# korneelvdbroek/audiocodec

Measured on AMD Instinct MI355X. Metric: MDCT frames/s (48 kHz, N=1024) encode+decode, higher is better.
Workload: dtype f32

## Files before the change

audiocodec_amd/csrc/ac_fast_inv.hip:

```cpp
#include "ac_fast_inv_dev.h"

namespace ac {

int pick_seglen(long long pairs, int frames, int preferred) {
  static const int fixed = [] {
    const char* e = getenv("AC_SEGLEN");
    return e ? atoi(e) : 0;
  }();
  int s = fixed > 0 ? fixed : preferred;
  if (s > frames) s = frames;
  if (s < 1) s = 1;
  return s;
}

template <int R, int IOF>
static void launch_inv_R(const InvArgs& a, int C, unsigned grid, hipStream_t s) {
  const dim3 blk(AC_WAVES * 64);
  if (C == 2) hipLaunchKernelGGL((k_inv_fast<R, 0, AC_WAVES, IOF>), dim3(grid), blk, 0, s, a);
  else if (C == 1) hipLaunchKernelGGL((k_inv_fast<R, 2, AC_WAVES, IOF>), dim3(grid), blk, 0, s, a);
  else if constexpr (IOF != 2) hipLaunchKernelGGL((k_inv_fast<R, 1, AC_WAVES, IOF>), dim3(grid), blk, 0, s, a);
}

int launch_inv_fast(const ac_mdct_plan* p, const float* X, void* x, int iof, const float* tail_in, float* tail_out,
                    int B, int Kp, int nblk, int C, hipStream_t s) {
  if (B <= 0 || C <= 0 || nblk <= 0) return AC_OK;
  if (fast_mdct_frames_per_wave(p->N) > 1) {
    if (!fast_multi_serves(p, C, iof, Kp)) {
      set_error("internal: no wave-level synthesis kernel for filters_n = %d, %d channels, io format %d here", p->N, C, iof);
      return AC_EUNSUPPORTED;
    }
    return launch_inv_multi(p, X, x, iof, tail_in, tail_out, B, Kp, nblk, C, s);
  }
  InvArgs a;
  unsigned grid;
  const int st = prep_inv_fast(p, X, x, iof, tail_in, tail_out, B, Kp, nblk, C, a, grid);
  if (st) return st;
  if (p->N == Geo<8>::FN) {
    if (iof == 2) launch_inv_R<8, 2>(a, C, grid, s);
    else if (iof == 1) launch_inv_R<8, 1>(a, C, grid, s);
    else launch_inv_R<8, 0>(a, C, grid, s);
  } else if (iof == 2) launch_inv_R<16, 2>(a, C, grid, s);
  else if (iof == 1) launch_inv_R<16, 1>(a, C, grid, s);
  else launch_inv_R<16, 0>(a, C, grid, s);
  AC_HIP_CHECK(hipGetLastError());
  return AC_OK;
}

bool fast_inv_quant_serves(const ac_mdct_plan* p, int C) {
  return p->fast && fast_mdct_frames_per_wave(p->N) == 1 && (C == 1 || C == 2);
}

template <int R, int IOF>
static void launch_inv_q_R(const InvArgs& a, const QuantRows& qr, int C, unsigned grid, hipStream_t s) {
  const dim3 blk(AC_WAVES * 64);
  if (C == 2) hipLaunchKernelGGL((k_inv_fast_q<R, 0, AC_WAVES, IOF>), dim3(grid), blk, 0, s, a, qr);
  else hipLaunchKernelGGL((k_inv_fast_q<R, 2, AC_WAVES, IOF>), dim3(grid), blk, 0, s, a, qr);
}

int launch_inv_fast_quant(const ac_mdct_plan* p, const ac_psy_plan* psy, const int16_t* codes, const int8_t* sf, void* x,
                          bool pcm16, int B, int Kp, int C, hipStream_t s) {
  if (B <= 0 || C <= 0 || Kp <= 0) return AC_OK;
  if (!fast_inv_quant_serves(p, C) || psy->N != p->N) {
    set_error("internal: no synthesis from quantised spectra for filters_n = %d, %d channels", p->N, C);
    return AC_EUNSUPPORTED;
  }
  InvArgs a;
  unsigned grid;
  const int st = prep_inv_fast(p, reinterpret_cast<const float*>(codes), x, pcm16 ? 1 : 0, nullptr, nullptr, B, Kp, Kp + 1, C,
                               a, grid);
  if (st) return st;
  QuantRows qr;
  qr.sf = sf;
  qr.band32 = reinterpret_cast<const uint32_t*>(psy->d_qband);
  qr.M = psy->M;
  if (p->N == Geo<8>::FN) {
    if (pcm16) launch_inv_q_R<8, 4>(a, qr, C, grid, s);
    else launch_inv_q_R<8, 3>(a, qr, C, grid, s);
  } else if (pcm16) launch_inv_q_R<16, 4>(a, qr, C, grid, s);
  else launch_inv_q_R<16, 3>(a, qr, C, grid, s);
  AC_HIP_CHECK(hipGetLastError());
  return AC_OK;
}

}
```

audiocodec_amd/csrc/ac_fast_inv_dev.h:

```cpp
#pragma once
#include <cstdlib>

#include "ac_fast.h"
#include "ac_fast_dev.h"

namespace ac {
namespace {

struct InvArgs {
  const float* X;
  void* x;
  const float* tail_in;
  float* tail_out;
  const float* tab;
  int B, Kp, nblk, C, seglen, nseg;
  int rev;
  long long npairs, nsig;
  long long ntasks;
};

template <int R>
__device__ __forceinline__ void idct_frame(const v4f (&frm)[R], char* buf, gtab_t tab, const v2f (&p1)[R], int lane,
                                           v2f (&now)[R], v2f (&nxt)[R]) {
  using G = Geo<R>;
  C2 z[R];
  {
    v2f xo_in[R], xo[R];
#pragma unroll
    for (int c = 0; c < R; ++c) xo_in[c] = v2f{frm[c].z, frm[c].w};
    rev_exchange<R - 1, R>(buf, lane, xo_in, xo);
#pragma unroll
    for (int r = 0; r < R; ++r) {
      const C2 v = {v2f{frm[r].x, frm[r].y}, xo[r]};
      z[r] = cmul(v, reinterpret_cast<const v2f*>(tab + G::I_PRE)[r * 64 + lane]);
    }
  }
  fft_wave<R>(z, buf, tab, p1, lane);
#pragma unroll
  for (int j = 0; j < R; ++j) {
    const C2 r = cmul_negim(z[j], reinterpret_cast<const v2f*>(tab + G::I_POST)[j * 64 + lane]);
    if (j < R / 2) {
      now[j] = r.re;
      nxt[j] = r.im;
    } else {
      now[j] = r.im;
      nxt[j] = r.re;
    }
  }
}

struct QuantRows {
  const int8_t* sf;
  const uint32_t* band32;
  int M;
};

template <int R, int CMODE, int NW, int IOF = 0>
__device__ __forceinline__ void inv_fast_body(const InvArgs& a, char* lds, const int bid, const int nblocks,
                                              const QuantRows* qr = nullptr) {
  using G = Geo<R>;
  constexpr bool QUANT = IOF >= 3;
  constexpr int OIOF = QUANT ? IOF - 3 : IOF;
  constexpr int FH = G::FH;
  const int lane = threadIdx.x & 63, wave = __builtin_amdgcn_readfirstlane(threadIdx.x >> 6);
  load_tables<NW, WAVE_LDS, G::I_LDS, 0>(lds, a.tab + G::I_TOTAL, nullptr);
  char* buf = lds + wave * WAVE_LDS;
  gtab_t tab = reinterpret_cast<const float*>(lds + NW * WAVE_LDS);
  v2f p1[R];
  load_p1<R>(a.tab + G::I_TOTAL, lane, p1);
  const int C = a.C;
  const size_t blk = (size_t)G::FN * C;
  constexpr bool COOP = (R == 8);
  const long long task_raw = (long long)(a.rev ? nblocks - 1 - bid : bid) * NW + wave;
  const bool valid = task_raw < a.ntasks;
  const long long task = valid ? task_raw : a.ntasks - 1;
  const int sgm = (int)(task % a.nseg);
  const Pair pq = make_pair<CMODE>(task / a.nseg, C, a.nsig);
  const bool has1 = pq.has1;
  const int n0 = sgm * a.seglen;
  const int n1 = min(a.nblk, n0 + a.seglen);
  using spec_t = typename std::conditional<IOF == 2 || QUANT, int16_t, float>::type;
  const spec_t* X0 = reinterpret_cast<const spec_t*>(a.X) + row_off(pq.b0, a.Kp, 0, blk, pq.c0);
  const spec_t* X1 = reinterpret_cast<const spec_t*>(a.X) + row_off(pq.b1, a.Kp, 0, blk, pq.c1);
  using hold_t = typename std::conditional<QUANT, QGran, v4f>::type;
  constexpr bool BW_REGS = QUANT && R == 8;
  uint32_t bw[BW_REGS ? R : 1];
  if constexpr (BW_REGS) {
#pragma unroll
    for (int i = 0; i < R; ++i) bw[i] = qr->band32[64 * i + lane];
  }
  auto load_frame = [&](int n, const spec_t* r0, const spec_t* r1, hold_t (&dst)[R]) {
    if constexpr (QUANT) {
      const size_t mc = (size_t)qr->M * C;
      const int8_t* sf0 = qr->sf + row_off(pq.b0, a.Kp, n, mc, pq.c0);
      const int8_t* sf1 = qr->sf + row_off(pq.b1, a.Kp, n, mc, pq.c1);
      if constexpr (BW_REGS) {
        load_row_q<CMODE, R>(r0, r1, sf0, sf1, bw, has1, lane, dst);
      } else {
        uint32_t bl[R];
#pragma unroll
        for (int i = 0; i < R; ++i) bl[i] = qr->band32[64 * i + lane];
        load_row_q<CMODE, R>(r0, r1, sf0, sf1, bl, has1, lane, dst);
      }
    } else if constexpr (IOF == 2) load_row_h<Bf16Fmt, CMODE, R>(r0, r1, C, has1, lane, dst);
    else load_row<CMODE, R>(r0, r1, C, has1, lane, dst);
  };
  const size_t ts0 = ((size_t)pq.b0 * C + pq.c0) * FH, ts1 = ((size_t)pq.b1 * C + pq.c1) * FH;
  constexpr bool AHEAD = (R == 8);
  const bool left = valid && n0 >= 1;
  const bool deferred = COOP && left && wave > 0;

  auto emit = [&](int n, const v2f (&now)[R], const v2f (&cin)[R]) {
    v4f row[R];
    v2f xe[R], xo_in[R], xo[R];
#pragma unroll
    for (int j2 = 0; j2 < R; ++j2) {
      const v2f ab = reinterpret_cast<const v2f*>(tab + G::I_COEF)[j2 * 64 + lane];
      const v2f o1 = ab.x * now[j2] + ab.y * cin[j2];
      const v2f o2 = ab.y * now[j2] - ab.x * cin[j2];
      xe[(j2 + R / 2) & (R - 1)] = (j2 < R / 2) ? o2 : o1;
      xo_in[j2] = (j2 < R / 2) ? o1 : o2;
    }
    rev_exchange<R / 2 - 1, R>(buf, lane, xo_in, xo);
#pragma unroll
    for (int i = 0; i < R; ++i) row[i] = v4f{xe[i].x, xe[i].y, xo[i].x, xo[i].y};
    const size_t o0 = row_off(pq.b0, a.nblk, n, blk, pq.c0), o1 = row_off(pq.b1, a.nblk, n, blk, pq.c1);
    if constexpr (OIOF != 0)
      store_row_h<typename RowFmt<OIOF>::type, CMODE, R>(static_cast<int16_t*>(a.x) + o0, static_cast<int16_t*>(a.x) + o1, C, has1, lane, row);
    else store_row<CMODE, R>(static_cast<float*>(a.x) + o0, static_cast<float*>(a.x) + o1, C, has1, lane, row);
  };

  v2f carry[R], now0[R];
#pragma unroll
  for (int r = 0; r < R; ++r) {
    carry[r] = v2f{0.f, 0.f};
    now0[r] = v2f{0.f, 0.f};
  }
  if (valid) {
    hold_t ahead[R];
    if (left && !deferred) {
      hold_t row[R];
      load_frame(n0 - 1, X0 + (size_t)(n0 - 1) * blk, X1 + (size_t)(n0 - 1) * blk, row);
      if (AHEAD && n0 < a.Kp) load_frame(n0, X0 + (size_t)n0 * blk, X1 + (size_t)n0 * blk, ahead);
      v2f dummy[R];
      if constexpr (QUANT) {
        v4f frm[R];
        dequant_frame<R>(row, frm);
        idct_frame<R>(frm, buf, tab, p1, lane, dummy, carry);
      } else {
        idct_frame<R>(row, buf, tab, p1, lane, dummy, carry);
      }
    } else {
      if (AHEAD && n0 < a.Kp) load_frame(n0, X0 + (size_t)n0 * blk, X1 + (size_t)n0 * blk, ahead);
      if (!left && a.tail_in) {
#pragma unroll
        for (int j2 = 0; j2 < R; ++j2) {
          const int k = lane + 64 * j2;
          const int j = (j2 < R / 2) ? (FH - 1 - 2 * k) : (2 * k - FH);
          carry[j2].x = a.tail_in[ts0 + j];
          carry[j2].y = has1 ? a.tail_in[ts1 + j] : 0.f;
        }
      }
    }

    for (int n = n0; n < n1; ++n) {
      v2f now[R], nxt[R];
      if (n < a.Kp) {
        if (!AHEAD) load_frame(n, X0 + (size_t)n * blk, X1 + (size_t)n * blk, ahead);
        if constexpr (QUANT) {
          v4f frm[R];
          dequant_frame<R>(ahead, frm);
          idct_frame<R>(frm, buf, tab, p1, lane, now, nxt);
        } else {
          idct_frame<R>(ahead, buf, tab, p1, lane, now, nxt);
        }
        if (AHEAD && n + 1 < n1 && n + 1 < a.Kp)
          load_frame(n + 1, X0 + (size_t)(n + 1) * blk, X1 + (size_t)(n + 1) * blk, ahead);
      } else {
#pragma unroll
        for (int r = 0; r < R; ++r) {
          now[r] = v2f{0.f, 0.f};
          nxt[r] = v2f{0.f, 0.f};
        }
      }
      if (deferred && n == n0) {
#pragma unroll
        for (int r = 0; r < R; ++r) now0[r] = now[r];
      } else {
        emit(n, now, carry);
      }
#pragma unroll
      for (int r = 0; r < R; ++r) carry[r] = nxt[r];
    }

    if (a.tail_out && n1 == a.nblk) {
#pragma unroll
      for (int j2 = 0; j2 < R; ++j2) {
        const int k = lane + 64 * j2;
        const int j = (j2 < R / 2) ? (FH - 1 - 2 * k) : (2 * k - FH);
        a.tail_out[ts0 + j] = carry[j2].x;
        if (has1) a.tail_out[ts1 + j] = carry[j2].y;
      }
    }
  }

  if (COOP) {
    wave_sync();
    if (valid) {
#pragma unroll
      for (int r = 0; r < R; ++r) *reinterpret_cast<v2f*>(buf + 8 * lane + 512 * r) = carry[r];
    }
    __syncthreads();
    v2f cin[R];
    if (deferred) {
#pragma unroll
      for (int r = 0; r < R; ++r) cin[r] = *reinterpret_cast<const v2f*>(buf - WAVE_LDS + 8 * lane + 512 * r);
    }
    __syncthreads();
    if (deferred) emit(n0, now0, cin);
  }
}

template <int R, int CMODE, int NW, int IOF = 0>
__global__ __launch_bounds__(NW * 64, ((IOF == 2 || (IOF == 1 && !(R == 8 && CMODE != 1))) ? 2 : wpe<R, CMODE>())) void k_inv_fast(InvArgs a) {
  __shared__ __attribute__((aligned(16))) char lds[NW * WAVE_LDS + Geo<R>::TAB_LDS];
  inv_fast_body<R, CMODE, NW, IOF>(a, lds, (int)blockIdx.x, (int)gridDim.x);
}

template <int R, int CMODE, int NW, int IOF>
__global__ __launch_bounds__(NW * 64, 2) void k_inv_fast_q(InvArgs a, QuantRows qr) {
  static_assert(IOF == 3 || IOF == 4, "quantised spectra");
  __shared__ __attribute__((aligned(16))) char lds[NW * WAVE_LDS + Geo<R>::TAB_LDS];
  inv_fast_body<R, CMODE, NW, IOF>(a, lds, (int)blockIdx.x, (int)gridDim.x, &qr);
}

static int prep_inv_fast(const ac_mdct_plan* p, const float* X, void* x, int iof, const float* tail_in, float* tail_out,
                         int B, int Kp, int nblk, int C, InvArgs& a, unsigned& grid) {
  if (iof == 2 && C > 2) {
    set_error("internal: no wave-level synthesis kernel for bfloat16 tensors with %d channels", C);
    return AC_EUNSUPPORTED;
  }
  a.X = X;
  a.x = x;
  a.tail_in = tail_in;
  a.tail_out = tail_out;
  a.tab = p->d_fast;
  a.B = B;
  a.Kp = Kp;
  a.nblk = nblk;
  a.C = C;
  a.nsig = (long long)B * C;
  a.npairs = (C == 2) ? (long long)B : (a.nsig + 1) / 2;
  a.seglen = pick_seglen(a.npairs, nblk, (p->N == Geo<8>::FN && C == 2) ? 2 : 3);
  if (a.npairs * ((nblk + a.seglen - 1) / a.seglen) < (long long)AC_WAVES * p->cus * 2) a.seglen = pick_seglen(a.npairs, nblk, 1);
  a.nseg = (nblk + a.seglen - 1) / a.seglen;
  a.ntasks = a.npairs * a.nseg;
  static const int inv_rev = [] { const char* e = getenv("AC_INV_REV"); return e ? atoi(e) : 0; }();
  a.rev = inv_rev;
  return grid_for(a.ntasks, AC_WAVES, &grid);
}

}
}
```

Before: 284.6 million.

## Let inverse MDCT blocks loop over several task rounds with carry hand-off

Each workgroup of the N=1024 inverse kernel now processes T rounds of tasks. The overlap carry of the last wave is handed to wave 0 of the next round through LDS, so wave 0 can skip recomputing the previous frame. The goal is to amortise table loading and the redundant left-frame IDCT across rounds, using a smaller grid. With the default of one round, behaviour is essentially unchanged apart from the restructured loop, extra registers (hand, pinned p1) and asm barriers.

```diff
diff --git a/audiocodec_amd/csrc/ac_fast_inv.hip b/audiocodec_amd/csrc/ac_fast_inv.hip
--- a/audiocodec_amd/csrc/ac_fast_inv.hip
+++ b/audiocodec_amd/csrc/ac_fast_inv.hip
@@ -11,6 +11,17 @@
   if (s > frames) s = frames;
   if (s < 1) s = 1;
   return s;
+}
+
+constexpr int INV_ROUNDS = 1;
+static int set_inv_rounds(const ac_mdct_plan* p, InvArgs& a, unsigned& grid) {
+  if (p->N != Geo<8>::FN) return AC_OK;
+  const char* e = getenv("AC_INV_ROUNDS");
+  int T = e ? atoi(e) : 0;
+  if (T <= 0) T = INV_ROUNDS;
+  if (T > 64) T = 64;
+  a.T = T;
+  return grid_for((a.ntasks + T - 1) / T, AC_WAVES, &grid);
 }
 
 template <int R, int IOF>
@@ -33,7 +44,8 @@
   }
   InvArgs a;
   unsigned grid;
-  const int st = prep_inv_fast(p, X, x, iof, tail_in, tail_out, B, Kp, nblk, C, a, grid);
+  int st = prep_inv_fast(p, X, x, iof, tail_in, tail_out, B, Kp, nblk, C, a, grid);
+  if (!st) st = set_inv_rounds(p, a, grid);
   if (st) return st;
   if (p->N == Geo<8>::FN) {
     if (iof == 2) launch_inv_R<8, 2>(a, C, grid, s);
@@ -66,8 +78,8 @@
   }
   InvArgs a;
   unsigned grid;
-  const int st = prep_inv_fast(p, reinterpret_cast<const float*>(codes), x, pcm16 ? 1 : 0, nullptr, nullptr, B, Kp, Kp + 1, C,
-                               a, grid);
+  int st = prep_inv_fast(p, reinterpret_cast<const float*>(codes), x, pcm16 ? 1 : 0, nullptr, nullptr, B, Kp, Kp + 1, C, a, grid);
+  if (!st) st = set_inv_rounds(p, a, grid);
   if (st) return st;
   QuantRows qr;
   qr.sf = sf;
diff --git a/audiocodec_amd/csrc/ac_fast_inv_dev.h b/audiocodec_amd/csrc/ac_fast_inv_dev.h
--- a/audiocodec_amd/csrc/ac_fast_inv_dev.h
+++ b/audiocodec_amd/csrc/ac_fast_inv_dev.h
@@ -15,9 +15,15 @@
   const float* tab;
   int B, Kp, nblk, C, seglen, nseg;
   int rev;
+  int T;
   long long npairs, nsig;
   long long ntasks;
 };
+
+template <typename V>
+__device__ __forceinline__ void per_round(V& v) {
+  asm volatile("" : "+v"(v));
+}
 
 template <int R>
 __device__ __forceinline__ void idct_frame(const v4f (&frm)[R], char* buf, gtab_t tab, const v2f (&p1)[R], int lane,
@@ -62,7 +68,8 @@
   constexpr bool QUANT = IOF >= 3;
   constexpr int OIOF = QUANT ? IOF - 3 : IOF;
   constexpr int FH = G::FH;
-  const int lane = threadIdx.x & 63, wave = __builtin_amdgcn_readfirstlane(threadIdx.x >> 6);
+  int lane = threadIdx.x & 63;
+  const int wave = __builtin_amdgcn_readfirstlane(threadIdx.x >> 6);
   load_tables<NW, WAVE_LDS, G::I_LDS, 0>(lds, a.tab + G::I_TOTAL, nullptr);
   char* buf = lds + wave * WAVE_LDS;
   gtab_t tab = reinterpret_cast<const float*>(lds + NW * WAVE_LDS);
@@ -71,17 +78,12 @@
   const int C = a.C;
   const size_t blk = (size_t)G::FN * C;
   constexpr bool COOP = (R == 8);
-  const long long task_raw = (long long)(a.rev ? nblocks - 1 - bid : bid) * NW + wave;
-  const bool valid = task_raw < a.ntasks;
-  const long long task = valid ? task_raw : a.ntasks - 1;
-  const int sgm = (int)(task % a.nseg);
-  const Pair pq = make_pair<CMODE>(task / a.nseg, C, a.nsig);
-  const bool has1 = pq.has1;
-  const int n0 = sgm * a.seglen;
-  const int n1 = min(a.nblk, n0 + a.seglen);
+  const int T = COOP ? a.T : 1;
+  const long long first = (long long)(a.rev ? nblocks - 1 - bid : bid) * (NW * T);
+  const int nmine = (int)min(a.ntasks - first, (long long)(NW * T));
+  const long long pair0 = first / a.nseg;
+  const unsigned sgm0 = (unsigned)(first - pair0 * a.nseg);
   using spec_t = typename std::conditional<IOF == 2 || QUANT, int16_t, float>::type;
-  const spec_t* X0 = reinterpret_cast<const spec_t*>(a.X) + row_off(pq.b0, a.Kp, 0, blk, pq.c0);
-  const spec_t* X1 = reinterpret_cast<const spec_t*>(a.X) + row_off(pq.b1, a.Kp, 0, blk, pq.c1);
   using hold_t = typename std::conditional<QUANT, QGran, v4f>::type;
   constexpr bool BW_REGS = QUANT && R == 8;
   uint32_t bw[BW_REGS ? R : 1];
@@ -89,135 +91,179 @@
 #pragma unroll
     for (int i = 0; i < R; ++i) bw[i] = qr->band32[64 * i + lane];
   }
-  auto load_frame = [&](int n, const spec_t* r0, const spec_t* r1, hold_t (&dst)[R]) {
-    if constexpr (QUANT) {
-      const size_t mc = (size_t)qr->M * C;
-      const int8_t* sf0 = qr->sf + row_off(pq.b0, a.Kp, n, mc, pq.c0);
-      const int8_t* sf1 = qr->sf + row_off(pq.b1, a.Kp, n, mc, pq.c1);
-      if constexpr (BW_REGS) {
-        load_row_q<CMODE, R>(r0, r1, sf0, sf1, bw, has1, lane, dst);
+  constexpr bool AHEAD = (R == 8);
+  auto pin_p1 = [&]() {
+    if constexpr (COOP) {
+#pragma unroll
+      for (int k = 1; k < R; ++k) per_round(p1[k]);
+    }
+  };
+  v2f hand[R];
+#pragma unroll
+  for (int r = 0; r < R; ++r) hand[r] = v2f{0.f, 0.f};
+
+  for (int t = 0; t < T; ++t) {
+    per_round(lane);
+    const int mine = t * NW + wave;
+    const bool valid = mine < nmine;
+    const unsigned ofs = sgm0 + (unsigned)(valid ? mine : nmine - 1);
+    const unsigned dp = ofs / (unsigned)a.nseg;
+    const int sgm = (int)(ofs - dp * (unsigned)a.nseg);
+    const Pair pq = make_pair<CMODE>(pair0 + dp, C, a.nsig);
+    const bool has1 = pq.has1;
+    const int n0 = sgm * a.seglen;
+    const int n1 = min(a.nblk, n0 + a.seglen);
+    const spec_t* X0 = reinterpret_cast<const spec_t*>(a.X) + row_off(pq.b0, a.Kp, 0, blk, pq.c0);
+    const spec_t* X1 = reinterpret_cast<const spec_t*>(a.X) + row_off(pq.b1, a.Kp, 0, blk, pq.c1);
+    auto load_frame = [&](int n, const spec_t* r0, const spec_t* r1, hold_t (&dst)[R]) {
+      if constexpr (QUANT) {
+        const size_t mc = (size_t)qr->M * C;
+        const int8_t* sf0 = qr->sf + row_off(pq.b0, a.Kp, n, mc, pq.c0);
+        const int8_t* sf1 = qr->sf + row_off(pq.b1, a.Kp, n, mc, pq.c1);
+        if constexpr (BW_REGS) {
+          load_row_q<CMODE, R>(r0, r1, sf0, sf1, bw, has1, lane, dst);
+        } else {
+          uint32_t bl[R];
+#pragma unroll
+          for (int i = 0; i < R; ++i) bl[i] = qr->band32[64 * i + lane];
+          load_row_q<CMODE, R>(r0, r1, sf0, sf1, bl, has1, lane, dst);
+        }
+      } else if constexpr (IOF == 2) load_row_h<Bf16Fmt, CMODE, R>(r0, r1, C, has1, lane, dst);
+      else load_row<CMODE, R>(r0, r1, C, has1, lane, dst);
+    };
+    const size_t ts0 = ((size_t)pq.b0 * C + pq.c0) * FH, ts1 = ((size_t)pq.b1 * C + pq.c1) * FH;
+    const bool left = valid && n0 >= 1;
+    const bool deferred = COOP && left && wave > 0;
+    const bool handed = COOP && left && wave == 0 && t > 0;
+
+    auto emit = [&](int n, const v2f (&now)[R], const v2f (&cin)[R]) {
+      v4f row[R];
+      v2f xe[R], xo_in[R], xo[R];
+#pragma unroll
+      for (int j2 = 0; j2 < R; ++j2) {
+        const v2f ab = reinterpret_cast<const v2f*>(tab + G::I_COEF)[j2 * 64 + lane];
+        const v2f o1 = ab.x * now[j2] + ab.y * cin[j2];
+        const v2f o2 = ab.y * now[j2] - ab.x * cin[j2];
+        xe[(j2 + R / 2) & (R - 1)] = (j2 < R / 2) ? o2 : o1;
+        xo_in[j2] = (j2 < R / 2) ? o1 : o2;
+      }
+      rev_exchange<R / 2 - 1, R>(buf, lane, xo_in, xo);
+#pragma unroll
+      for (int i = 0; i < R; ++i) row[i] = v4f{xe[i].x, xe[i].y, xo[i].x, xo[i].y};
+      const size_t o0 = row_off(pq.b0, a.nblk, n, blk, pq.c0), o1 = row_off(pq.b1, a.nblk, n, blk, pq.c1);
+      if constexpr (OIOF != 0)
+        store_row_h<typename RowFmt<OIOF>::type, CMODE, R>(static_cast<int16_t*>(a.x) + o0, static_cast<int16_t*>(a.x) + o1, C, has1, lane, row);
+      else store_row<CMODE, R>(static_cast<float*>(a.x) + o0, static_cast<float*>(a.x) + o1, C, has1, lane, row);
+    };
+
+    v2f carry[R], now0[R];
+#pragma unroll
+    for (int r = 0; r < R; ++r) {
+      carry[r] = v2f{0.f, 0.f};
+      now0[r] = v2f{0.f, 0.f};
+    }
+    const bool extra = left && !deferred && !handed;
+    hold_t ahead[R], row[R];
+#pragma unroll
+    for (int i = 0; i < R; ++i) {
+      ahead[i] = hold_t{};
+      row[i] = hold_t{};
+    }
+    if (valid) {
+      if (extra) load_frame(n0 - 1, X0 + (size_t)(n0 - 1) * blk, X1 + (size_t)(n0 - 1) * blk, row);
+      if (AHEAD && n0 < a.Kp) load_frame(n0, X0 + (size_t)n0 * blk, X1 + (size_t)n0 * blk, ahead);
+    }
+    if (valid) {
+      if (extra) {
+        v2f dummy[R];
+        if constexpr (QUANT) {
+          v4f frm[R];
+          dequant_frame<R>(row, frm);
+          idct_frame<R>(frm, buf, tab, p1, lane, dummy, carry);
+        } else {
+          idct_frame<R>(row, buf, tab, p1, lane, dummy, carry);
+        }
       } else {
-        uint32_t bl[R];
-#pragma unroll
-        for (int i = 0; i < R; ++i) bl[i] = qr->band32[64 * i + lane];
-        load_row_q<CMODE, R>(r0, r1, sf0, sf1, bl, has1, lane, dst);
-      }
-    } else if constexpr (IOF == 2) load_row_h<Bf16Fmt, CMODE, R>(r0, r1, C, has1, lane, dst);
-    else load_row<CMODE, R>(r0, r1, C, has1, lane, dst);
-  };
-  const size_t ts0 = ((size_t)pq.b0 * C + pq.c0) * FH, ts1 = ((size_t)pq.b1 * C + pq.c1) * FH;
-  constexpr bool AHEAD = (R == 8);
-  const bool left = valid && n0 >= 1;
-  const bool deferred = COOP && left && wave > 0;
-
-  auto emit = [&](int n, const v2f (&now)[R], const v2f (&cin)[R]) {
-    v4f row[R];
-    v2f xe[R], xo_in[R], xo[R];
-#pragma unroll
-    for (int j2 = 0; j2 < R; ++j2) {
-      const v2f ab = reinterpret_cast<const v2f*>(tab + G::I_COEF)[j2 * 64 + lane];
-      const v2f o1 = ab.x * now[j2] + ab.y * cin[j2];
-      const v2f o2 = ab.y * now[j2] - ab.x * cin[j2];
-      xe[(j2 + R / 2) & (R - 1)] = (j2 < R / 2) ? o2 : o1;
-      xo_in[j2] = (j2 < R / 2) ? o1 : o2;
-    }
-    rev_exchange<R / 2 - 1, R>(buf, lane, xo_in, xo);
-#pragma unroll
-    for (int i = 0; i < R; ++i) row[i] = v4f{xe[i].x, xe[i].y, xo[i].x, xo[i].y};
-    const size_t o0 = row_off(pq.b0, a.nblk, n, blk, pq.c0), o1 = row_off(pq.b1, a.nblk, n, blk, pq.c1);
-    if constexpr (OIOF != 0)
-      store_row_h<typename RowFmt<OIOF>::type, CMODE, R>(static_cast<int16_t*>(a.x) + o0, static_cast<int16_t*>(a.x) + o1, C, has1, lane, row);
-    else store_row<CMODE, R>(static_cast<float*>(a.x) + o0, static_cast<float*>(a.x) + o1, C, has1, lane, row);
-  };
-
-  v2f carry[R], now0[R];
-#pragma unroll
-  for (int r = 0; r < R; ++r) {
-    carry[r] = v2f{0.f, 0.f};
-    now0[r] = v2f{0.f, 0.f};
-  }
-  if (valid) {
-    hold_t ahead[R];
-    if (left && !deferred) {
-      hold_t row[R];
-      load_frame(n0 - 1, X0 + (size_t)(n0 - 1) * blk, X1 + (size_t)(n0 - 1) * blk, row);
-      if (AHEAD && n0 < a.Kp) load_frame(n0, X0 + (size_t)n0 * blk, X1 + (size_t)n0 * blk, ahead);
-      v2f dummy[R];
-      if constexpr (QUANT) {
-        v4f frm[R];
-        dequant_frame<R>(row, frm);
-        idct_frame<R>(frm, buf, tab, p1, lane, dummy, carry);
-      } else {
-        idct_frame<R>(row, buf, tab, p1, lane, dummy, carry);
-      }
-    } else {
-      if (AHEAD && n0 < a.Kp) load_frame(n0, X0 + (size_t)n0 * blk, X1 + (size_t)n0 * blk, ahead);
-      if (!left && a.tail_in) {
+        if (handed) {
+#pragma unroll
+          for (int r = 0; r < R; ++r) carry[r] = hand[r];
+        } else if (!left && a.tail_in) {
+#pragma unroll
+          for (int j2 = 0; j2 < R; ++j2) {
+            const int k = lane + 64 * j2;
+            const int j = (j2 < R / 2) ? (FH - 1 - 2 * k) : (2 * k - FH);
+            carry[j2].x = a.tail_in[ts0 + j];
+            carry[j2].y = has1 ? a.tail_in[ts1 + j] : 0.f;
+          }
+        }
+      }
+
+      for (int n = n0; n < n1; ++n) {
+        v2f now[R], nxt[R];
+        if (n < a.Kp) {
+          if (!AHEAD) load_frame(n, X0 + (size_t)n * blk, X1 + (size_t)n * blk, ahead);
+          pin_p1();
+          if constexpr (QUANT) {
+            v4f frm[R];
+            dequant_frame<R>(ahead, frm);
+            idct_frame<R>(frm, buf, tab, p1, lane, now, nxt);
+          } else {
+            idct_frame<R>(ahead, buf, tab, p1, lane, now, nxt);
+          }
+          if (AHEAD && n + 1 < n1 && n + 1 < a.Kp)
+            load_frame(n + 1, X0 + (size_t)(n + 1) * blk, X1 + (size_t)(n + 1) * blk, ahead);
+        } else {
+#pragma unroll
+          for (int r = 0; r < R; ++r) {
+            now[r] = v2f{0.f, 0.f};
+            nxt[r] = v2f{0.f, 0.f};
+          }
+        }
+        if (deferred && n == n0) {
+#pragma unroll
+          for (int r = 0; r < R; ++r) now0[r] = now[r];
+        } else {
+          emit(n, now, carry);
+        }
+#pragma unroll
+        for (int r = 0; r < R; ++r) carry[r] = nxt[r];
+      }
+
+      if (a.tail_out && n1 == a.nblk) {
 #pragma unroll
         for (int j2 = 0; j2 < R; ++j2) {
           const int k = lane + 64 * j2;
           const int j = (j2 < R / 2) ? (FH - 1 - 2 * k) : (2 * k - FH);
-          carry[j2].x = a.tail_in[ts0 + j];
-          carry[j2].y = has1 ? a.tail_in[ts1 + j] : 0.f;
-        }
-      }
-    }
-
-    for (int n = n0; n < n1; ++n) {
-      v2f now[R], nxt[R];
-      if (n < a.Kp) {
-        if (!AHEAD) load_frame(n, X0 + (size_t)n * blk, X1 + (size_t)n * blk, ahead);
-        if constexpr (QUANT) {
-          v4f frm[R];
-          dequant_frame<R>(ahead, frm);
-          idct_frame<R>(frm, buf, tab, p1, lane, now, nxt);
-        } else {
-          idct_frame<R>(ahead, buf, tab, p1, lane, now, nxt);
-        }
-        if (AHEAD && n + 1 < n1 && n + 1 < a.Kp)
-          load_frame(n + 1, X0 + (size_t)(n + 1) * blk, X1 + (size_t)(n + 1) * blk, ahead);
+          a.tail_out[ts0 + j] = carry[j2].x;
+          if (has1) a.tail_out[ts1 + j] = carry[j2].y;
+        }
+      }
+    }
+
+    if (COOP) {
+      wave_sync();
+      if (valid) {
+#pragma unroll
+        for (int r = 0; r < R; ++r) *reinterpret_cast<v2f*>(buf + 8 * lane + 512 * r) = carry[r];
+      }
+      __syncthreads();
+      v2f cin[R];
+#pragma unroll
+      for (int r = 0; r < R; ++r) cin[r] = v2f{0.f, 0.f};
+      if (deferred) {
+#pragma unroll
+        for (int r = 0; r < R; ++r) cin[r] = *reinterpret_cast<const v2f*>(buf - WAVE_LDS + 8 * lane + 512 * r);
+      }
+      if (t + 1 < T) {
+#pragma unroll
+        for (int r = 0; r < R; ++r) hand[r] = *reinterpret_cast<const v2f*>(lds + (NW - 1) * WAVE_LDS + 8 * lane + 512 * r);
       } else {
 #pragma unroll
-        for (int r = 0; r < R; ++r) {
-          now[r] = v2f{0.f, 0.f};
-          nxt[r] = v2f{0.f, 0.f};
-        }
-      }
-      if (deferred && n == n0) {
-#pragma unroll
-        for (int r = 0; r < R; ++r) now0[r] = now[r];
-      } else {
-        emit(n, now, carry);
-      }
-#pragma unroll
-      for (int r = 0; r < R; ++r) carry[r] = nxt[r];
-    }
-
-    if (a.tail_out && n1 == a.nblk) {
-#pragma unroll
-      for (int j2 = 0; j2 < R; ++j2) {
-        const int k = lane + 64 * j2;
-        const int j = (j2 < R / 2) ? (FH - 1 - 2 * k) : (2 * k - FH);
-        a.tail_out[ts0 + j] = carry[j2].x;
-        if (has1) a.tail_out[ts1 + j] = carry[j2].y;
-      }
-    }
-  }
-
-  if (COOP) {
-    wave_sync();
-    if (valid) {
-#pragma unroll
-      for (int r = 0; r < R; ++r) *reinterpret_cast<v2f*>(buf + 8 * lane + 512 * r) = carry[r];
-    }
-    __syncthreads();
-    v2f cin[R];
-    if (deferred) {
-#pragma unroll
-      for (int r = 0; r < R; ++r) cin[r] = *reinterpret_cast<const v2f*>(buf - WAVE_LDS + 8 * lane + 512 * r);
-    }
-    __syncthreads();
-    if (deferred) emit(n0, now0, cin);
+        for (int r = 0; r < R; ++r) hand[r] = v2f{0.f, 0.f};
+      }
+      __syncthreads();
+      if (deferred) emit(n0, now0, cin);
+    }
   }
 }
 
@@ -257,6 +303,7 @@
   a.ntasks = a.npairs * a.nseg;
   static const int inv_rev = [] { const char* e = getenv("AC_INV_REV"); return e ? atoi(e) : 0; }();
   a.rev = inv_rev;
+  a.T = 1;
   return grid_for(a.ntasks, AC_WAVES, &grid);
 }
 
```

Result: no change. 284.3 million (median of 3 runs) (-0.1%).
